# szbonaldo/FedMLP

Measured on AMD Instinct MI355X. Metric: images/sec/client (ICH 224x224 bs=128) at 1/2/4/8 GPUs; mAP vs ref, higher is better.
Workload: dtype f32; 1 GPU; FedMLP stage1 step, Resnet18, ICH-shaped synthetic 3x224x224, C=5, bs=128, one client per GPU, FedAvg all-reduce every 40 steps + once at end; parallelism=clients1, rccl_ranks=1, stream_mode=default: frozen teacher + weight gradients on the engine's side stream, arithmetic=fp32 operands+sums; products as 6 exact bf16 partials on the bf16 matrix pipe

## Files before the change

fedmlp_amd/_lib.py:

```python
import ctypes as C
import os

_HERE = os.path.dirname(os.path.abspath(__file__))
LIB_PATH = os.environ.get("FEDMLP_HIP_LIB") or os.path.join(_HERE, "libfedmlp_hip.so")

FM_MAX_CLASSES = 32
FM_COMM_ID_BYTES = 128


class FmConfig(C.Structure):
    _fields_ = [("model", C.c_int32), ("n_classes", C.c_int32), ("in_h", C.c_int32),
                ("in_w", C.c_int32), ("max_images", C.c_int32), ("reserved", C.c_int32 * 3),
                ("stream", C.c_void_p)]


class FmAdam(C.Structure):
    _fields_ = [("lr", C.c_float), ("beta1", C.c_float), ("beta2", C.c_float),
                ("eps", C.c_float), ("weight_decay", C.c_float)]


_P = C.c_void_p
_F = C.POINTER(C.c_float)
_I32 = C.c_int32
_I64 = C.c_int64
# ... 50 lines not shown
    "fm_profile_read": (C.c_int, [_P, _I32, C.POINTER(_I64), C.POINTER(C.c_double),
                                  C.POINTER(C.c_double)]),
    "fm_comm_preflight": (C.c_int, []),
    "fm_comm_unique_id": (C.c_int, [C.POINTER(C.c_uint8)]),
    "fm_comm_init": (C.c_int, [_P, C.POINTER(C.c_uint8), _I32, _I32]),
    "fm_comm_destroy": (C.c_int, [_P]),
    "fm_comm_size": (C.c_int, [_P]),
    "fm_fedavg_allreduce": (C.c_int, [_P, C.c_float]),
    "fm_fedavg_tao": (C.c_int, [_P, C.POINTER(C.c_double), C.c_double, _F, C.POINTER(C.c_double)]),
    "fm_fedavg_proto": (C.c_int, [_P, _P, C.c_double, _F, _P]),
    "fm_profile_ops": (C.c_int, [_P, _I32, C.c_char_p, _I32]),
    "fm_debug_num_convs": (C.c_int, [_P]),
    "fm_debug_conv_info": (C.c_int, [_P, _I32, C.POINTER(_I32)]),
    "fm_debug_conv": (C.c_int, [_P, _I32, _I32, _P, _P, _P, _I32, _I32, _P]),
    "fm_debug_block_dgrad": (C.c_int, [_P, _I32, _P, _P, _P, _I32]),
    "fm_debug_pw": (C.c_int, [_P, _I32, _I32, _P, _P, _P, _I32, _I32, _P, _P, _P, _P]),
    "fm_debug_proj_bwd": (C.c_int, [_P, _I32, _I32, _P, _P, _P, _P, _P, _I32, _I32, _P, _P]),
    "fm_debug_exp_bwd": (C.c_int, [_P, _I32, _P, _P, _P, _P, _P, _I32, _I32, _P, _P]),
    "fm_debug_get_grads": (C.c_int, [_P, _P]),
    "fm_debug_activation": (C.c_int, [_P, _I32, _I32, _I32, _P, C.POINTER(_I32)]),
    "fm_debug_stem_masks": (C.c_int, [_P, _I32, _I32, _P, _P]),
    "fm_debug_lose_part": (C.c_int, [_I32]),
    "fm_debug_ew": (C.c_int, [_P, _I32, C.POINTER(_P), C.POINTER(_I32), _F]),
    "fm_debug_eff": (C.c_int, [_P, _I32, C.POINTER(_P), C.POINTER(_I32), _F]),
    "fm_debug_eff_ws": (C.c_int, [_I32, C.POINTER(_I32), C.POINTER(C.c_int64)]),
}

_lib = None


# ... 39 lines not shown
```

fedmlp_amd/csrc/common.h:

```cpp
#pragma once
#include <hip/hip_runtime.h>
#include <stdint.h>

#include <stdlib.h>

typedef float f32x4 __attribute__((ext_vector_type(4)));

#ifndef FM_F32_FAST_SWISH
#define FM_F32_FAST_SWISH 1
#endif
#ifdef __HIPCC__
__device__ __forceinline__ float fm_swish_f32(float v)
{
#if FM_F32_FAST_SWISH
    return v * __builtin_amdgcn_rcpf(1.f + __expf(-v));
#else
    return v / (1.f + expf(-v));
#endif
}
#endif


#ifndef FM_MFMA_SPLIT_DEFAULT
#define FM_MFMA_SPLIT_DEFAULT 6
// ... 112 lines not shown
    int sp = 0;
    const unsigned short* Wsp = nullptr;
    const unsigned short* Xp = nullptr;
    long long xp_pix = 0;
    unsigned short* Yp = nullptr;
    long long yp_pix = 0;
    const unsigned short* resp = nullptr;
    int wrow = 0;
    int lose_part = 0;
    int* err = nullptr;
    int* err_host = nullptr;
    int njobs = 0;
    PconvJob job[PCONV_MAX_JOBS];
    const unsigned short* Xp2 = nullptr;
    unsigned wsp_bytes = 0;
};
void pconv_debug_lose_part(int on);

struct WgradParams {
    const float* dY;
    const float* X;
    float* slab;
    const int4* tab;
    const float* zeros;
    int M, Nw;
    int Ho, Wo, Hi, Wi, Ci, stride;
    int npix;
    int pix_per_split;
    int tilesM, tilesN;
    int bn;
// ... 23 lines not shown
    float* stats;
    int imgs, imgs_per_group, Hp, Wp, Ho, Wo, relu, sp;
    long long plane_bytes;
};
bool stem_rows_takes(int k, int stride, int cout, int hout, int wout, long long plane_bytes);
int stem_rows_stats_tiles(int imgs_per_group, int hout);
void launch_stem_rows(StemRowsParams p, hipStream_t s);
void k_stem_weight_planes(const float* w, unsigned short* dst, int Kw, hipStream_t s);
int launch_pwgrad(PwgradParams p, size_t slab_floats, hipStream_t s);
bool pwgrad_ring_takes(const PwgradParams& p);
int launch_pwgrad_ring(PwgradParams p, size_t slab_floats, hipStream_t s);
bool pwgrad_takes(int M, int Ci, int ksz, long long npix, long long xpix, int Wi, int pad);
void launch_igemm(IgemmParams p, int groups, hipStream_t s);
void launch_pconv(IgemmParams p, int groups, hipStream_t s);
bool pconv_takes(int M, int Ci, long long xp_pix, int Wi);
bool pconv_uses_ts(const IgemmParams& p);
int pconv_tile_m(int M);
int pconv_tile_n(int M);
size_t pconv_slab_floats();
bool launch_conv1x1_stream(const IgemmParams& p, int groups, hipStream_t s);
bool conv1x1_stream_takes(int Ci, int M, int Co);
int igemm_max_blocks();
bool launch_wgrad(const WgradParams& p, int splits, hipStream_t s);
int wgrad_tile_n(int M, int Nw);
int launch_wgrad_skinny(const WgradParams& p, size_t slab_floats, hipStream_t s);
int igemm_tile_n(int M, bool stem = false);
int igemm_tile_m(int M);

#include <stdio.h>
inline void set_max_dyn_lds(const void* fn, int bytes, const char* what)
// ... 5 lines not shown
```

fedmlp_amd/csrc/engine.hip:

```cpp
#include <math.h>
#include <stdio.h>
#include <string.h>

#include <algorithm>
#include <string>
#include <vector>

#include "../../include/fedmlp_hip.h"
#include "../../include/fedmlp_hip_debug.h"
#include "comm.h"
#include "common.h"
#include "kernels.h"
#include "pwconv.h"

static thread_local std::string g_err;
const char* fm_last_error(void) { return g_err.c_str(); }
const char* fm_version(void) { return "fedmlp_hip 0.2 (gfx950)"; }

#define HIPCHK(x)                                                                              \
    do {                                                                                       \
        hipError_t e_ = (x);                                                                   \
        if (e_ != hipSuccess) {                                                                \
            char b_[512];                                                                      \
            snprintf(b_, sizeof b_, "%s:%d %s -> %s", __FILE__, __LINE__, #x, hipGetErrorString(e_)); \
// ... 141 lines not shown
    size_t NP = 0, NS = 0;
    size_t off_fcw = 0, off_fcb = 0, off_gamma = 0, off_beta = 0, off_rm = 0, off_rv = 0;
    int64_t nf_sd = 0, ni_sd = 0;
    float *grad = nullptr, *adam_m = nullptr, *adam_v = nullptr;
    float* stage_sd = nullptr;
    fm_adam hp{3e-5f, 0.9f, 0.999f, 1e-8f, 5e-4f};
    int64_t adam_t = 0;
    float *x4 = nullptr, *dyh0 = nullptr;
    float* x3 = nullptr;
    bool stem_rows = false;
    unsigned short* x3p = nullptr;
    long long x3p_plane_elems = 0;
    uint8_t* idx0 = nullptr;
    float *GA = nullptr, *GB = nullptr, *GC = nullptr, *GD = nullptr, *GE = nullptr;
    float *ws_stats = nullptr, *ws_part = nullptr;
    int stats_conv = -1, stats_tiles_n = 0;
    size_t slab_floats = 0;
    float *ca = nullptr, *cb = nullptr, *cc = nullptr;
    float *feat = nullptr, *logits = nullptr, *tfeat = nullptr, *tlogits = nullptr, *dlogits = nullptr;
    float* psum = nullptr;
    int64_t *pcnt = nullptr, *tcnt = nullptr;
    float* zeros = nullptr;
    int *sel_counts = nullptr, *sel_top = nullptr, *sel_bot = nullptr, *cls_dev = nullptr;
    int sel_cap = 0;
    int* tag_buf = nullptr;
    size_t tag_buf_ints = 0;
    bool prof = false, prof_fail = false;
    hipError_t soft_err = hipSuccess;
    int* dev_err = nullptr;
    int* host_err = nullptr;
    int* host_err_dev = nullptr;
// ... 652 lines not shown
    const Conv& c0 = e->convs[0];
    if (e->model == 0) {
        const size_t pooled = B * (c0.hout / 2) * (c0.wout / 2) * 64;
        DALLOC(e->idx0, pooled);
        DALLOC(e->dyh0, B * c0.hout * c0.wout * 64);
        DALLOC(e->GA, pooled); DALLOC(e->GB, pooled); DALLOC(e->GC, pooled); DALLOC(e->GD, pooled); DALLOC(e->GE, pooled);
    } else {
        const EffSizes z = eff_sizes(e);
        AALLOC(e->GA, z.g_io); AALLOC(e->GB, z.g_io);
        AALLOC(e->T_small, z.t_small); AALLOC(e->T_big, z.t_big);
        DALLOC(e->se_dgp, B * z.max_ce); DALLOC(e->se_drp, B * z.max_cs); DALLOC(e->se_ds, B * z.max_ce);
        side = side && side_fits(e);
        DALLOC(e->hfeat, B * e->D);
    }
    DALLOC(e->ws_stats, max_stats);
    DALLOC(e->ws_part, (size_t)2 * (1024 + 32) * 2 * e->maxC);
    e->slab_floats = std::max<size_t>(max_slab * 8, (size_t)48 << 20);
    DALLOC(e->main.ws_slab, e->slab_floats);
    e->main.rec = e->main.ws_slab;
    DALLOC(e->ca, 2 * e->maxC); DALLOC(e->cb, 2 * e->maxC); DALLOC(e->cc, 2 * e->maxC);
    DALLOC(e->feat, B * e->D); DALLOC(e->tfeat, B * e->D);
    DALLOC(e->logits, B * e->C); DALLOC(e->tlogits, B * e->C); DALLOC(e->dlogits, B * e->C);
    DALLOC(e->psum, (size_t)2 * e->C * e->D); DALLOC(e->pcnt, 2 * e->C); DALLOC(e->tcnt, e->C);
    DALLOC(e->sel_counts, 2); DALLOC(e->cls_dev, FM_MAX_CLASSES);
    DALLOC(e->zeros, 64);
    if (e->planes) {
        const size_t pooled = B * (c0.hout / 2) * (c0.wout / 2) * 64;
        PALLOC(e->GBp, pooled); PALLOC(e->GCp, pooled); PALLOC(e->GDp, pooled);
        size_t mx = 0;
        for (auto& c : e->convs) {
            if (c.cin == 3) continue;
// ... 177 lines not shown
    p.imgs_per_group = imgs / groups;
    p.tilesM = (c.cout_p + igemm_tile_m(c.cout_p) - 1) / igemm_tile_m(c.cout_p);
    const int bn = igemm_tile_n(c.cout_p, c.cin == 3);
    p.tilesN = (p.imgs_per_group * c.hout * c.wout + bn - 1) / bn;
    p.relu = relu;
    ProfScope ps(e, L, c.cin == 3 ? 2 : (c.cout_p >= 128 ? 0 : 1), 2.0 * c.macs_per_img * imgs);
    launch_igemm(p, groups, L.st);
}

int stats_tiles(fm_engine* e, int ci)
{
    if (e->stats_conv != ci) soft(e, hipErrorInvalidValue);
    return e->stats_tiles_n;
}

void conv_dgrad(fm_engine* e, Lane& L, int ci, const float* dy, float* dx, int imgs, const float* res,
                bool acc_cls0, const unsigned short* dyp = nullptr)
{
    Conv& c = e->convs[ci];
    if (e->planes && c.ncls > 0 && c.cls[0].bm_off >= 0 &&
        pconv_takes(c.cin_p, c.cout_p, (long long)imgs * c.hout * c.wout, c.wout)) {
        const long long xp_pix = (long long)imgs * c.hout * c.wout;
        if (!dyp) dyp = scratch_planes(e, L, dy, xp_pix, c.cout_p);
        for (int k = 0; k < c.ncls; ++k) {
            DgradClass& d = c.cls[k];
            IgemmParams p{};
            p.Xp = dyp; p.xp_pix = xp_pix; p.Wsp = e->wbm_d + d.bm_off;
            p.Y = dx; p.slab = L.sk_slab; p.counters = L.sk_counters; p.err = e->dev_err; p.err_host = e->host_err_dev; p.sp = e->products;
            p.ntaps = d.taps.n;
            for (int t = 0; t < d.taps.n; ++t) { p.dh[t] = d.dh[t]; p.dw[t] = d.dw[t]; }
            p.res = res ? res : ((acc_cls0 && d.ph == 0 && d.pw == 0) ? dx : nullptr);
            p.M = c.cin_p;
            p.Hi = c.hout; p.Wi = c.wout; p.Ci = c.cout_p;
            p.Hg = (c.hin - d.ph + c.stride - 1) / c.stride;
            p.Wg = (c.win - d.pw + c.stride - 1) / c.stride;
            p.sg = 1;
            p.Ho = c.hin; p.Wo = c.win; p.Co = c.cin_p;
            p.os = c.stride; p.oh0 = d.ph; p.ow0 = d.pw;
            p.imgs_per_group = imgs;
            p.tilesM = c.cin_p / pconv_tile_m(c.cin_p);
            p.tilesN = (imgs * p.Hg * p.Wg + pconv_tile_n(c.cin_p) - 1) / pconv_tile_n(c.cin_p);
            p.relu = 0;
            ProfScope ps(e, L, (c.cin_p >= 128 ? 0 : 1) + (pconv_uses_ts(p) ? 0 : 6), 2.0 * c.macs_per_img * imgs * d.taps.n / (double)(c.k * c.k));
            launch_pconv(p, 1, L.st);
        }
        return;
    }
    if (e->planes && c.cin != 3) { soft(e, hipErrorInvalidValue); return; }
    if (e->precision && c.k == 1) {
        PwParams q{};
        q.zeros = e->zeros;
        q.W = e->student.wb + c.wbt_off;
        q.X = reinterpret_cast<const bf16*>(dy); q.Y = reinterpret_cast<bf16*>(dx);
        q.M = c.cin_p; q.K = c.cout_p;
        q.npix = imgs * c.hout * c.wout; q.groups = 1;
        q.res = reinterpret_cast<const bf16*>(res);
        q.HW = c.hout * c.wout;
        launch_pw_conv(q, L.st);
        return;
// ... 166 lines not shown
void bn_fwd_finalize(fm_engine* e, Lane& L, int ci, int groups, int imgs_per_group, BnMode mode)
{
    const Conv& c = e->convs[ci];
    const int bi = c.bn;
    Bn& b = e->bns[bi];
    if (mode == BnMode::Frozen) { bn_fwd_fixed(e, L, b, groups); return; }
    const bool run = mode == BnMode::Batch;
    k_bn_finalize(e->ws_stats, groups, stats_tiles(e, ci), b.C, imgs_per_group * c.hout * c.wout,
                  e->student.state + e->off_gamma + b.ch_off, e->student.state + e->off_beta + b.ch_off,
                  run ? e->student.state + e->off_rm + b.ch_off : nullptr, run ? e->student.state + e->off_rv + b.ch_off : nullptr, b.mean,
                  b.istd, b.scale, b.shift, e->bn_eps, e->bn_mom, L.st, e->dev_err);
    if (run) e->student.counters[bi] += groups;
}

void bn_bwd(fm_engine* e, Lane& L, int bi, const float* dz, const float* z, float* dy, float* dyh_out, int groups,
            int imgs_per_group, bool frozen, bool z_is_relu_of_bn = false, unsigned short* dyp = nullptr, const unsigned short* zh = nullptr)
{
    const Conv& c = e->convs[bi];
    Bn& b = e->bns[bi];
    const int pix = imgs_per_group * c.hout * c.wout;
    const char* fy = getenv("FM_BN_MASK_FROM_Y");
    const int from_y = fy ? atoi(fy) : 1;
    const float *msc = nullptr, *msh = nullptr;
    if (z_is_relu_of_bn && (z || zh) && (from_y || !z)) { msc = b.scale; msh = b.shift; z = nullptr; zh = nullptr; }
    k_bn_bwd_reduce(dz, z, c.y, b.mean, b.istd, e->ws_part, groups, pix, b.C, L.st, msc, msh, zh);
    k_bn_bwd_finalize(e->ws_part, groups, bn_bwd_blocks(pix), b.C, pix, e->student.state + e->off_gamma + b.ch_off, b.mean,
                      b.istd, e->ca, e->cb, e->cc, e->grad + e->off_gamma + b.ch_off,
                      e->grad + e->off_beta + b.ch_off, L.st, frozen);
    if (dyp) k_bn_bwd_apply_planes(dz, z, c.y, e->ca, e->cb, e->cc, dy, dyp, dyh_out, groups, pix, b.C, L.st, msc, msh, zh);
    else k_bn_bwd_apply(dz, z, c.y, e->ca, e->cb, e->cc, dy, dyh_out, groups, pix, b.C, L.st, msc, msh);
}

void to_nhwc4(fm_engine* e, Lane& L, const float* const* xs, int groups, int B)
{
    if (e->precision && e->model == 1) {
        const Conv& c = e->convs[e->c_stem];
        for (int g = 0; g < groups; ++g)
            k_stem_im2col(xs[g], reinterpret_cast<bf16*>(e->stem_col) + (size_t)g * B * c.hout * c.wout * c.Kw, B, e->H, e->W, c.hout,
                          c.wout, c.k, c.stride, c.pad, c.pad, L.st);
        return;
    }
// ... 215 lines not shown
    unsigned short* PB[2] = {e->GBp, sw ? e->GB2p : e->GBp};
    unsigned short* PC[2] = {e->GCp, sw ? e->GC2p : e->GCp};
    unsigned short* PD[2] = {e->GDp, sw ? e->GD2p : e->GDp};
    k_fc_bwd(e->dlogits, e->feat, S + e->off_fcw, nullptr, e->grad + e->off_fcw, e->grad + e->off_fcb, e->GA, DT_F32, imgs,
             512, e->C, cl.hout * cl.wout, L.st, bw.dfeat);
    float *ga = e->GA, *ge = e->GE;
    for (int b = (int)e->blocks.size() - 1; b >= 0; --b) {
        const Block& blk = e->blocks[b];
        const BlockActs& a = A.blk[b];
        const int par = b & 1;
        float *GB = GBp[par], *GC = GCp[par], *GD = GDp[par];
        unsigned short *gbp = pm ? PB[par] : nullptr, *gcp = pm ? PC[par] : nullptr, *gdp = pm ? PD[par] : nullptr;
        const float* in = b == 0 ? A.p0 : A.blk[b - 1].out;
        const bool last = b + 1 == (int)e->blocks.size();
        side_guard(e, 0, par);
        if (pm && !last) bn_bwd(e, L, blk.c2, ga, nullptr, nullptr, ga, groups, B, bw.frozen, false, gbp, a.outp);
        else bn_bwd(e, L, blk.c2, ga, a.out, pm ? nullptr : GB, ga, groups, B, bw.frozen, false, gbp);
        if (blk.ds >= 0) { side_guard(e, 1, par); bn_bwd(e, L, blk.ds, ga, nullptr, pm ? nullptr : GC, nullptr, groups, B, bw.frozen, false, gcp); }
        side_guard(e, 2, par);
        conv_dgrad(e, L, blk.c2, GB, GD, imgs, nullptr, false, gbp);
        conv_wgrad(e, side_begin(e, 0, par), blk.c2, a.z1, GB, imgs, nullptr, 0, pm ? a.z1p : nullptr, gbp);
        side_end(e, 0, par);
        if (pm) bn_bwd(e, L, blk.c1, GD, nullptr, nullptr, nullptr, groups, B, bw.frozen, true, gdp, a.z1p);
        else bn_bwd(e, L, blk.c1, GD, a.z1, GD, nullptr, groups, B, bw.frozen, true);
        if (blk.ds >= 0) {
            if (!block_dgrad(e, L, blk.c1, blk.ds, GD, GC, ge, imgs, gdp, gcp)) {
                conv_dgrad(e, L, blk.ds, GC, ge, imgs, nullptr, false, gcp);
                conv_dgrad(e, L, blk.c1, GD, ge, imgs, nullptr, true, gdp);
            }
        } else {
            conv_dgrad(e, L, blk.c1, GD, ge, imgs, ga, false, gdp);
        }
        const unsigned short* inp = pm ? (b == 0 ? A.p0p : A.blk[b - 1].outp) : nullptr;
        conv_wgrad(e, side_begin(e, 2, par), blk.c1, in, GD, imgs, nullptr, 0, inp, gdp);
        side_end(e, 2, par);
        if (blk.ds >= 0) {
            conv_wgrad(e, side_begin(e, 1, par), blk.ds, in, GC, imgs, nullptr, 0, inp, gcp);
            side_end(e, 1, par);
        }
        std::swap(ga, ge);
    }
    const Conv& c0 = e->convs[0];
    {
        Bn& b0 = e->bns[0];
// ... 1333 lines not shown
int fm_debug_block_dgrad(fm_engine* e, int32_t block, const float* dy1_dev, const float* dyd_dev, float* dx_dev, int32_t imgs)
{
    ARGCHK(e && dy1_dev && dyd_dev && dx_dev, "null tensor");
    ARGCHK(e->model == 0 && !e->precision, "fm_debug_block_dgrad: a precision-0 ResNet-18 engine");
    ARGCHK(block >= 0 && block < (int)e->blocks.size() && e->blocks[block].ds >= 0, "block has no downsample");
    ARGCHK(imgs >= 1 && imgs <= e->maxB, "imgs");
    ensure_packed(e);
    const Block& blk = e->blocks[block];
    if (!block_dgrad(e, e->main, blk.c1, blk.ds, dy1_dev, dyd_dev, dx_dev, imgs)) {
        conv_dgrad(e, e->main, blk.ds, dyd_dev, dx_dev, imgs, nullptr, false);
        conv_dgrad(e, e->main, blk.c1, dy1_dev, dx_dev, imgs, nullptr, true);
    }
    return FM_OK;
}

int fm_debug_conv_info(fm_engine* e, int32_t conv, int32_t* info16)
{
    ARGCHK(e && info16 && conv >= 0 && conv < (int)e->convs.size(), "conv index");
    const Conv& c = e->convs[conv];
    const int v[16] = {c.cin, c.cout, c.k, c.stride, c.pad, c.hin, c.win, c.hout, c.wout, c.cin_p, c.Kw, c.kw_p,
                       c.cout_p, 0, 0, 0};
    memcpy(info16, v, sizeof v);
    return FM_OK;
}

int fm_debug_conv(fm_engine* e, int32_t op, int32_t conv, const float* x_dev, const float* dy_dev, float* out_dev,
                  int32_t imgs, int32_t groups, float* stats_dev)
{
    ARGCHK(e && out_dev && conv >= 0 && conv < (int)e->convs.size(), "conv index");
    ARGCHK(!e->precision, "fm_debug_conv works on fp32 tensors: create the engine with precision 0");
// ... 264 lines not shown
```

fedmlp_amd/csrc/pconv.hip:

```cpp
#include <stdlib.h>

#include <algorithm>
#include <type_traits>

#include "common.h"
#include "kernels.h"
#include "split3.h"

#if __HIP_DEVICE_COMPILE__
template <int IMM> __device__ __forceinline__ sp_u32x4 pc_lds_read128(unsigned addr)
{
    sp_u32x4 v;
    asm volatile("ds_read_b128 %0, %1 offset:%2" : "=v"(v) : "v"(addr), "n"(IMM));
    return v;
}
__device__ __forceinline__ void pc_divmod(int x, int d, float rcp, int& q, int& r)
{
    q = (int)((float)x * rcp);
    r = x - q * d;
    if (r < 0) { --q; r += d; }
    else if (r >= d) { ++q; r -= d; }
}
template <int CTRL> __device__ __forceinline__ float pc_dpp(float v)
{
// ... 7 lines not shown
template <int SP> __device__ __forceinline__ f32x4 pc_mfma(const sp_u32x4 (&a)[3], const sp_u32x4 (&b)[3], f32x4 v)
{
    return mfma_split<SP>(a[0], a[1], a[2], b[0], b[1], b[2], v);
}
#endif

#ifdef PC_PHASES
__device__ unsigned long long pc_prof[256 * 8];
#define PC_T(i) do { const unsigned long long t_ = clock64(); pc_acc[i] += t_ - pc_t; pc_t = t_; } while (0)
#else
#define PC_T(i) do { } while (0)
#endif
#ifndef PC_WAVES_PER_EU
#define PC_WAVES_PER_EU 2
#endif
template <int FR, int FC, int NS, int SP, bool TS = false>
__global__ __launch_bounds__(512, PC_WAVES_PER_EU) void pconv_kernel(const IgemmParams p)
{
#if __HIP_DEVICE_COMPILE__
#ifdef PC_PHASES
    unsigned long long pc_acc[8] = {0, 0, 0, 0, 0, 0, 0, 0};
    unsigned long long pc_t = clock64();
#endif
    constexpr int WN = 4;
    constexpr int BM = 32 * FR, BN = 64 * FC;
    constexpr int GA = BM / 16, GB = TS ? (BN + 2 + 15) / 16 : BN / 16;
    constexpr int BROWS = 16 * GB;
    constexpr int SA = 3 * BM * 64, SB = 3 * BROWS * 64;
    constexpr int NSB = TS ? 2 : NS;
    static_assert(!TS || FC == 4, "tap-row sharing: 256-pixel tiles");
    constexpr int JA = (3 * GA + 7) / 8;
    constexpr int RGB = (GB + 7) / 8;
    static_assert(NS == 2 && FC == 4 && (FR == 2 || FR == 4), "two LDS stages, 256-pixel tiles, 64 or 128 rows");
    typedef __attribute__((address_space(3))) void lds_void;
    extern __shared__ __attribute__((aligned(16))) unsigned char smem[];
    const int tid = threadIdx.x;
    const int lane = tid & 63, wave = __builtin_amdgcn_readfirstlane(tid >> 6);
    const int wm = wave / WN, wn = wave % WN;
    const int li = lane & 15, lg = lane >> 4;
    const unsigned lds0 = (unsigned)(size_t)smem;
    const unsigned As = lds0, Bs = lds0 + NS * SA;

    const int Wi = p.Wi;
    struct JobV {
        int nsteps, ntaps, k2, icc2;
// ... 431 lines not shown
                            for (int c = 0; c < FC; ++c)
                                part[q][c] = *reinterpret_cast<const f32x4*>(src + (((r + q) * FC + c) * 512 + tid) * 4);
#pragma unroll
                        for (int q = 0; q < 2; ++q)
#pragma unroll
                            for (int c = 0; c < FC; ++c) acc[r + q][c] += part[q][c];
                    }
                }
            }
        }

        PC_T(5);
        if (do_epilogue) {
        const int mbase = m0 + wm * (16 * FR) + 4 * lg;
        const JobV J = jobv(cur.jb);
        if (p.stats) {
            float* red = fsmem;
#pragma unroll
            for (int r = 0; r < FR; ++r) {
                f32x4 s1 = {0.f, 0.f, 0.f, 0.f}, s2 = {0.f, 0.f, 0.f, 0.f};
#pragma unroll
                for (int c = 0; c < FC; ++c) {
                    s1 += acc[r][c];
                    s2 += acc[r][c] * acc[r][c];
                }
#pragma unroll
                for (int q = 0; q < 4; ++q) {
                    float u = s1[q], v = s2[q];
                    u += pc_dpp<0xB1>(u); v += pc_dpp<0xB1>(v);
                    u += pc_dpp<0x4E>(u); v += pc_dpp<0x4E>(v);
                    u += pc_dpp<0x12C>(u); v += pc_dpp<0x12C>(v);
// ... 17 lines not shown
                st[m0 + ch] = u;
                st[p.M + m0 + ch] = v;
            }
        }
        size_t opix[FC];
        bool ok[FC];
#pragma unroll
        for (int c = 0; c < FC; ++c) {
            const int n = n0 + wn * (16 * FC) + 16 * c + li;
            ok[c] = n < J.npix;
            int img, rem, hg, wg;
            pc_divmod(ok[c] ? n : J.npix - 1, J.HWg, J.rcpHW, img, rem);
            pc_divmod(rem, J.Wg, J.rcpW, hg, wg);
            opix[c] = (size_t)((grp * p.imgs_per_group + img) * p.Ho + hg * p.os + J.oh0) * p.Wo + (wg * p.os + J.ow0);
        }
#pragma unroll
        for (int r = 0; r < FR; r += 2) {
            __builtin_amdgcn_sched_barrier(0);
            const int m = mbase + 16 * r;
            const size_t cb = (size_t)(m0 + wm * (16 * FR) + 16 * r) >> 5;
            f32x4 sc0 = {1.f, 1.f, 1.f, 1.f}, sc1 = sc0, sh0 = {0.f, 0.f, 0.f, 0.f}, sh1 = sh0;
            if (p.scale) {
                sc0 = *reinterpret_cast<const f32x4*>(p.scale + m); sc1 = *reinterpret_cast<const f32x4*>(p.scale + m + 16);
                sh0 = *reinterpret_cast<const f32x4*>(p.shift + m); sh1 = *reinterpret_cast<const f32x4*>(p.shift + m + 16);
            }
#pragma unroll
            for (int c = 0; c < FC; ++c) {
                __builtin_amdgcn_sched_barrier(0);
                const size_t o = opix[c] * p.Co;
                f32x4 v0 = acc[r][c], v1 = acc[r + 1][c];
// ... 23 lines not shown
                }
                if (!ok[c]) continue;
                if (p.Y) {
                    *reinterpret_cast<f32x4*>(p.Y + o + m) = v0;
                    *reinterpret_cast<f32x4*>(p.Y + o + m + 16) = v1;
                }
                if (p.Yp) {
                    sp_u32x4 H, M, L;
                    split3(v0, v1, H, M, L);
                    unsigned char* dst = reinterpret_cast<unsigned char*>(p.Yp) + ((cb * 3) * (size_t)p.yp_pix + opix[c]) * 64 + lg * 16;
                    *reinterpret_cast<sp_u32x4*>(dst) = H;
                    *reinterpret_cast<sp_u32x4*>(dst + (size_t)p.yp_pix * 64) = M;
                    *reinterpret_cast<sp_u32x4*>(dst + (size_t)p.yp_pix * 128) = L;
                }
            }
        }
        }
        PC_T(6);
        if (!more) break;
        PC_SYNC_LDS();
        cur = nx;
    }
    if (pend_tile >= 0) {
        asm volatile("s_waitcnt vmcnt(0)" ::: "memory");
        __syncthreads();
        if (tid == 0) {
            __builtin_amdgcn_fence(__ATOMIC_RELEASE, "agent");
            asm volatile("s_waitcnt vmcnt(0)" ::: "memory");
            if (!p.lose_part) __hip_atomic_fetch_add(p.counters + pend_tile, 1, __ATOMIC_RELAXED, __HIP_MEMORY_SCOPE_AGENT);
        }
// ... 77 lines not shown
    return ((long long)(Ci >> 5) * 3 * xp_pix + Wi + 1) * 64 < 0x7ff00000LL && xp_pix < (1LL << 22);
}

bool pconv_uses_ts(const IgemmParams& p)
{
    bool ts = p.njobs == 0 && p.ntaps == 9 && p.sg == 1 && p.Hg == p.Hi && p.Wg == p.Wi;
    for (int j = 0; ts && j < 3; ++j) {
        ts = p.dh[3 * j] == p.dh[3 * j + 1] && p.dh[3 * j] == p.dh[3 * j + 2];
        int seen = 0;
        for (int k = 0; k < 3; ++k) seen |= 1 << (p.dw[3 * j + k] + 1);
        ts = ts && seen == 7;
    }
    return ts;
}

void launch_pconv(IgemmParams p, int groups, hipStream_t s)
{
    static bool attr_done = false;
    constexpr int LDS_L = 2 * 3 * (128 + 256) * 64 + 4 * 128 * 2 * 4;
    constexpr int LDS_S = 2 * 3 * (64 + 256) * 64 + 4 * 128 * 2 * 4;
    constexpr int LDS_LT = 2 * 3 * 128 * 64 + 2 * 3 * 272 * 64 + 4 * 128 * 2 * 4;
    constexpr int LDS_ST = 2 * 3 * 64 * 64 + 2 * 3 * 272 * 64 + 4 * 128 * 2 * 4;
    if (!attr_done) {
        set_max_dyn_lds(reinterpret_cast<const void*>(&pconv_kernel<4, 4, 2, 6, true>), LDS_LT, "pconv_kernel<4, 4, 2, 6, true>");
        set_max_dyn_lds(reinterpret_cast<const void*>(&pconv_kernel<4, 4, 2, 9, true>), LDS_LT, "pconv_kernel<4, 4, 2, 9, true>");
        set_max_dyn_lds(reinterpret_cast<const void*>(&pconv_kernel<2, 4, 2, 6, true>), LDS_ST, "pconv_kernel<2, 4, 2, 6, true>");
        set_max_dyn_lds(reinterpret_cast<const void*>(&pconv_kernel<2, 4, 2, 9, true>), LDS_ST, "pconv_kernel<2, 4, 2, 9, true>");
        set_max_dyn_lds(reinterpret_cast<const void*>(&pconv_kernel<4, 4, 2, 6>), LDS_L, "pconv_kernel<4, 4, 2, 6>");
        set_max_dyn_lds(reinterpret_cast<const void*>(&pconv_kernel<4, 4, 2, 9>), LDS_L, "pconv_kernel<4, 4, 2, 9>");
        set_max_dyn_lds(reinterpret_cast<const void*>(&pconv_kernel<2, 4, 2, 6>), LDS_S, "pconv_kernel<2, 4, 2, 6>");
        set_max_dyn_lds(reinterpret_cast<const void*>(&pconv_kernel<2, 4, 2, 9>), LDS_S, "pconv_kernel<2, 4, 2, 9>");
        attr_done = true;
    }
    const bool ts = pconv_uses_ts(p);
    p.tapcode = pconv_tapcode(p.dh, p.dw, p.ntaps);
    if (p.njobs == 0) {
        p.njobs = 1;
        PconvJob& j = p.job[0];
        j.ntaps = p.ntaps; j.tapcode = p.tapcode;
        j.cib = j.icc2 = p.Ci >> 5; j.wofs = j.wofs2 = 0;
        j.Hg = p.Hg; j.Wg = p.Wg; j.oh0 = p.oh0; j.ow0 = p.ow0;
    }
// ... 18 lines not shown
    p.tn_fast = p.tilesM > 1 && (long long)p.M * p.nsteps * 192 > (3LL << 20);
    static const int forced = getenv("FM_IGEMM_BLOCKS") ? atoi(getenv("FM_IGEMM_BLOCKS")) : 0;
    int nblk = p.total_steps >= 4LL * pconv_max_blocks() ? pconv_max_blocks() : (int)std::min<long long>(pconv_max_blocks(), T);
    if (forced > 0) nblk = (int)std::min<long long>(std::min(forced, pconv_max_blocks()), p.total_steps);
    p.steps_per_block = (int)((p.total_steps + nblk - 1) / nblk);
    if (forced <= 0 && p.steps_per_block > p.nsteps / 2 && (long long)p.nsteps * 128 * 192 > (2LL << 20)) {
        for (int P = 1; P <= 12; ++P) {
            if (p.nsteps % P) continue;
            const int q = p.nsteps / P;
            const int sq = (p.steps_per_block + q - 1) / q * q;
            if ((long long)sq * 100 <= (long long)p.steps_per_block * 102) { p.steps_per_block = sq; break; }
        }
    }
    dim3 grid(nblk);
    p.lose_part = g_lose_part ? 1 : 0;
    if (ts) {
        if (p.M >= 128) {
            if (p.sp == 9) hipLaunchKernelGGL((pconv_kernel<4, 4, 2, 9, true>), grid, dim3(512), LDS_LT, s, p);
            else hipLaunchKernelGGL((pconv_kernel<4, 4, 2, 6, true>), grid, dim3(512), LDS_LT, s, p);
        } else {
            if (p.sp == 9) hipLaunchKernelGGL((pconv_kernel<2, 4, 2, 9, true>), grid, dim3(512), LDS_ST, s, p);
            else hipLaunchKernelGGL((pconv_kernel<2, 4, 2, 6, true>), grid, dim3(512), LDS_ST, s, p);
        }
        return;
    }
    if (p.M >= 128) {
        if (p.sp == 9) hipLaunchKernelGGL((pconv_kernel<4, 4, 2, 9>), grid, dim3(512), LDS_L, s, p);
        else hipLaunchKernelGGL((pconv_kernel<4, 4, 2, 6>), grid, dim3(512), LDS_L, s, p);
    } else {
        if (p.sp == 9) hipLaunchKernelGGL((pconv_kernel<2, 4, 2, 9>), grid, dim3(512), LDS_S, s, p);
// ... 34 lines not shown
```

fedmlp_amd/engine.py:

```python
import ctypes as C

import numpy as np
import torch

from . import _lib, spec

MODEL_IDS = {"Resnet18": 0, "Efficient_b0": 1}
PRECISION_IDS = {"fp32": 0, "bf16": 1}
PRODUCT_FORMS = {None: 0, 6: 3, 0: 1, 9: 2}


def _ptr(t):
    if t is None:
        return None
    assert t.is_cuda and t.is_contiguous() and t.dtype in (torch.float32, torch.int32, torch.bfloat16), \
        (t.device, t.dtype, t.is_contiguous())
    return C.c_void_p(t.data_ptr())


class Engine:

    def __init__(self, model, n_classes, in_h, in_w, max_images, device=None, precision="fp32", streams=0, products=None):
        if not torch.cuda.is_available():
            raise RuntimeError("fedmlp_amd.Engine needs a GPU (no CPU fallback)")
# ... 433 lines not shown
        _lib.check(self.lib.fm_debug_activation(self.h, kind, block, imgs, out.ctypes.data_as(C.c_void_p), dims))
        return np.ascontiguousarray(out.transpose(0, 3, 1, 2))

    def debug_num_convs(self):
        return self.lib.fm_debug_num_convs(self.h)

    def debug_conv(self, op, conv, x, dy, out, imgs, groups=1, stats=None):
        self._enqueue()
        _lib.check(self.lib.fm_debug_conv(self.h, op, conv, _ptr(x), _ptr(dy), _ptr(out), imgs, groups,
                                          _ptr(stats)))

    def debug_block_dgrad(self, block, dy1, dyd, dx, imgs):
        self._enqueue()
        _lib.check(self.lib.fm_debug_block_dgrad(self.h, block, _ptr(dy1), _ptr(dyd), _ptr(dx), imgs))

    EW_OPS = ("split_planes", "planes_to_f32", "bn_finalize", "bn_finalize_frozen", "bn_eval_affine", "bn_apply",
              "bn_apply_planes", "stem_pool", "stem_pool_planes", "stem_pool_bwd", "stem_pool_bn_reduce", "stem_pool_bn_apply",
              "bn_bwd_reduce", "bn_bwd_finalize", "bn_bwd_apply", "bn_bwd_apply_planes")

    def debug_ew(self, op, ptrs, dims, scalars=()):
        assert len(ptrs) <= 12 and len(dims) <= 5 and len(scalars) <= 2, (len(ptrs), len(dims), len(scalars))
        for t in ptrs:
            assert t is None or (t.is_cuda and t.is_contiguous()), op
        p = (C.c_void_p * 12)(*[None if t is None else t.data_ptr() for t in ptrs])
        d = (C.c_int32 * 5)(*[int(v) for v in dims])
        _lib.check(self.lib.fm_debug_ew(self.h, self.EW_OPS.index(op), p, d, _lib.fvec(list(scalars) + [0.0] * (2 - len(scalars)))))

    EFF_OPS = ("dw_fwd", "dw_dgrad", "dw_wgrad", "se_fwd", "se_scale", "se_bwd_bn1", "se_wgrad")

    def debug_eff_ws(self, op, dims):
# ... 61 lines not shown
```

include/fedmlp_hip_debug.h:

```cpp
#ifndef FEDMLP_HIP_DEBUG_H
#define FEDMLP_HIP_DEBUG_H

#include "fedmlp_hip.h"

#ifdef __cplusplus
extern "C" {
#endif

int fm_debug_conv_info(fm_engine* e, int32_t conv, int32_t* info16);
int fm_debug_num_convs(fm_engine* e);
int fm_debug_conv(fm_engine* e, int32_t op, int32_t conv, const float* x_dev, const float* dy_dev,
                  float* out_dev, int32_t imgs, int32_t groups, float* stats_dev);

int fm_debug_block_dgrad(fm_engine* e, int32_t block, const float* dy1_dev, const float* dyd_dev, float* dx_dev, int32_t imgs);

int fm_debug_pw(fm_engine* e, int32_t op, int32_t conv, const void* x_dev, const void* dy_dev, void* out_dev,
                int32_t imgs, int32_t groups, const float* psc_dev, const float* psh_dev, const float* gate_dev,
                float* stats_dev);

int fm_debug_proj_bwd(fm_engine* e, int32_t conv, int32_t phase, const void* dyp_dev, const void* yd_dev, const float* bn_dev,
                      const float* gate_dev, const float* ds_dev, int32_t imgs, int32_t groups, void* out_dev,
                      float* pool5_dev);

int fm_debug_exp_bwd(fm_engine* e, int32_t conv, const void* da_dev, const void* ye_dev, const void* x_dev, const void* res_dev,
                     const float* bn_dev, int32_t imgs, int32_t groups, void* dx_dev, float* dw_dev);

int fm_debug_activation(fm_engine* e, int32_t kind, int32_t block, int32_t imgs, float* host_nhwc,
                        int32_t* dims4);

// ... 28 lines not shown
```

Measured before the change: 6174 images/sec.

## Fuse BatchNorm backward channel sums into tap-sharing dgrad epilogue

The planes-mode data-gradient convolution now computes, in its epilogue, the per-channel BatchNorm backward partial sums (sum of masked dz and sum of dz times normalized y) for the following BN layer and writes them to the partial workspace. The separate bn_bwd_reduce pass is then skipped, and finalize reads the tile-level partials. This removes one full read of the gradient and activation tensors per block, at the cost of extra loads and cross-lane reductions in the conv epilogue, more register pressure, and eight new kernel instantiations. Residual-add blocks take their ReLU mask from the stored planes.

```diff
diff --git a/fedmlp_amd/_lib.py b/fedmlp_amd/_lib.py
--- a/fedmlp_amd/_lib.py
+++ b/fedmlp_amd/_lib.py
@@ -88,6 +88,9 @@
     "fm_debug_conv_info": (C.c_int, [_P, _I32, C.POINTER(_I32)]),
     "fm_debug_conv": (C.c_int, [_P, _I32, _I32, _P, _P, _P, _I32, _I32, _P]),
     "fm_debug_block_dgrad": (C.c_int, [_P, _I32, _P, _P, _P, _I32]),
+    "fm_debug_dgrad_sums": (C.c_int, [_P, _I32, _I32, _I32, _P, _P, _P, _P, _P, _P, _P, _P, _P, _P, _I64, _I32, _I32,
+                                      C.POINTER(_I32)]),
+    "fm_debug_bn_sums": (C.c_int, [_P, _I32]),
     "fm_debug_pw": (C.c_int, [_P, _I32, _I32, _P, _P, _P, _I32, _I32, _P, _P, _P, _P]),
     "fm_debug_proj_bwd": (C.c_int, [_P, _I32, _I32, _P, _P, _P, _P, _P, _I32, _I32, _P, _P]),
     "fm_debug_exp_bwd": (C.c_int, [_P, _I32, _P, _P, _P, _P, _P, _I32, _I32, _P, _P]),
diff --git a/fedmlp_amd/csrc/common.h b/fedmlp_amd/csrc/common.h
--- a/fedmlp_amd/csrc/common.h
+++ b/fedmlp_amd/csrc/common.h
@@ -150,6 +150,14 @@
     PconvJob job[PCONV_MAX_JOBS];
     const unsigned short* Xp2 = nullptr;
     unsigned wsp_bytes = 0;
+    int bs_mode = 0;
+    const float* bs_y = nullptr;
+    const float* bs_mean = nullptr;
+    const float* bs_istd = nullptr;
+    const float* bs_msc = nullptr;
+    const float* bs_msh = nullptr;
+    const unsigned short* bs_zh = nullptr;
+    float* bs_part = nullptr;
 };
 void pconv_debug_lose_part(int on);
 
@@ -203,6 +211,7 @@
 void launch_igemm(IgemmParams p, int groups, hipStream_t s);
 void launch_pconv(IgemmParams p, int groups, hipStream_t s);
 bool pconv_takes(int M, int Ci, long long xp_pix, int Wi);
+bool pconv_takes_sums(const IgemmParams& p);
 bool pconv_uses_ts(const IgemmParams& p);
 int pconv_tile_m(int M);
 int pconv_tile_n(int M);
diff --git a/fedmlp_amd/csrc/engine.hip b/fedmlp_amd/csrc/engine.hip
--- a/fedmlp_amd/csrc/engine.hip
+++ b/fedmlp_amd/csrc/engine.hip
@@ -179,7 +179,10 @@
     uint8_t* idx0 = nullptr;
     float *GA = nullptr, *GB = nullptr, *GC = nullptr, *GD = nullptr, *GE = nullptr;
     float *ws_stats = nullptr, *ws_part = nullptr;
+    size_t ws_part_floats = 0;
     int stats_conv = -1, stats_tiles_n = 0;
+    int part_bn = -1, part_tiles_n = 0;
+    bool bn_sums = true;
     size_t slab_floats = 0;
     float *ca = nullptr, *cb = nullptr, *cc = nullptr;
     float *feat = nullptr, *logits = nullptr, *tfeat = nullptr, *tlogits = nullptr, *dlogits = nullptr;
@@ -862,7 +865,8 @@
         DALLOC(e->hfeat, B * e->D);
     }
     DALLOC(e->ws_stats, max_stats);
-    DALLOC(e->ws_part, (size_t)2 * (1024 + 32) * 2 * e->maxC);
+    e->ws_part_floats = (size_t)2 * (1024 + 32) * 2 * e->maxC;
+    DALLOC(e->ws_part, e->ws_part_floats);
     e->slab_floats = std::max<size_t>(max_slab * 8, (size_t)48 << 20);
     DALLOC(e->main.ws_slab, e->slab_floats);
     e->main.rec = e->main.ws_slab;
@@ -1070,10 +1074,26 @@
     return e->stats_tiles_n;
 }
 
+struct DgradSums {
+    int bn, groups;
+    const float *y, *mean, *istd, *msc, *msh;
+    const unsigned short* zh;
+    float* part;
+    size_t part_floats;
+};
+DgradSums dgrad_sums_for(fm_engine* e, int bi, int groups, const unsigned short* zh)
+{
+    const Bn& b = e->bns[bi];
+    return DgradSums{bi, groups, e->convs[bi].y, b.mean, b.istd, zh ? nullptr : b.scale, zh ? nullptr : b.shift, zh, e->ws_part,
+                     e->ws_part_floats};
+}
+int part_tiles(fm_engine* e, int bi) { return e->part_bn == bi ? e->part_tiles_n : 0; }
+
 void conv_dgrad(fm_engine* e, Lane& L, int ci, const float* dy, float* dx, int imgs, const float* res,
-                bool acc_cls0, const unsigned short* dyp = nullptr)
+                bool acc_cls0, const unsigned short* dyp = nullptr, const DgradSums* sums = nullptr)
 {
     Conv& c = e->convs[ci];
+    if (sums) e->part_bn = -1;
     if (e->planes && c.ncls > 0 && c.cls[0].bm_off >= 0 &&
         pconv_takes(c.cin_p, c.cout_p, (long long)imgs * c.hout * c.wout, c.wout)) {
         const long long xp_pix = (long long)imgs * c.hout * c.wout;
@@ -1097,8 +1117,23 @@
             p.tilesM = c.cin_p / pconv_tile_m(c.cin_p);
             p.tilesN = (imgs * p.Hg * p.Wg + pconv_tile_n(c.cin_p) - 1) / pconv_tile_n(c.cin_p);
             p.relu = 0;
+            int groups = 1;
+            if (sums && c.ncls == 1 && imgs % sums->groups == 0) {
+                IgemmParams q = p;
+                q.imgs_per_group = imgs / sums->groups;
+                q.tilesN = (q.imgs_per_group * p.Hg * p.Wg + pconv_tile_n(c.cin_p) - 1) / pconv_tile_n(c.cin_p);
+                q.bs_mode = sums->zh ? 2 : 1;
+                q.bs_y = sums->y; q.bs_mean = sums->mean; q.bs_istd = sums->istd; q.bs_part = sums->part;
+                q.bs_msc = sums->msc; q.bs_msh = sums->msh;
+                if (sums->zh) { q.bs_zh = sums->zh; q.yp_pix = (long long)imgs * c.hin * c.win; }
+                const size_t need = (size_t)sums->groups * (q.tilesN + (q.tilesN > 64 ? 32 : 0)) * 2 * c.cin_p;
+                if (need <= sums->part_floats && pconv_takes_sums(q)) {
+                    p = q; groups = sums->groups;
+                    e->part_bn = sums->bn; e->part_tiles_n = q.tilesN;
+                }
+            }
             ProfScope ps(e, L, (c.cin_p >= 128 ? 0 : 1) + (pconv_uses_ts(p) ? 0 : 6), 2.0 * c.macs_per_img * imgs * d.taps.n / (double)(c.k * c.k));
-            launch_pconv(p, 1, L.st);
+            launch_pconv(p, groups, L.st);
         }
         return;
     }
@@ -1295,7 +1330,8 @@
 }
 
 void bn_bwd(fm_engine* e, Lane& L, int bi, const float* dz, const float* z, float* dy, float* dyh_out, int groups,
-            int imgs_per_group, bool frozen, bool z_is_relu_of_bn = false, unsigned short* dyp = nullptr, const unsigned short* zh = nullptr)
+            int imgs_per_group, bool frozen, bool z_is_relu_of_bn = false, unsigned short* dyp = nullptr, const unsigned short* zh = nullptr,
+            int sums_ready = 0)
 {
     const Conv& c = e->convs[bi];
     Bn& b = e->bns[bi];
@@ -1304,8 +1340,9 @@
     const int from_y = fy ? atoi(fy) : 1;
     const float *msc = nullptr, *msh = nullptr;
     if (z_is_relu_of_bn && (z || zh) && (from_y || !z)) { msc = b.scale; msh = b.shift; z = nullptr; zh = nullptr; }
-    k_bn_bwd_reduce(dz, z, c.y, b.mean, b.istd, e->ws_part, groups, pix, b.C, L.st, msc, msh, zh);
-    k_bn_bwd_finalize(e->ws_part, groups, bn_bwd_blocks(pix), b.C, pix, e->student.state + e->off_gamma + b.ch_off, b.mean,
+    if (!sums_ready) k_bn_bwd_reduce(dz, z, c.y, b.mean, b.istd, e->ws_part, groups, pix, b.C, L.st, msc, msh, zh);
+    e->part_bn = -1;
+    k_bn_bwd_finalize(e->ws_part, groups, sums_ready ? sums_ready : bn_bwd_blocks(pix), b.C, pix, e->student.state + e->off_gamma + b.ch_off, b.mean,
                       b.istd, e->ca, e->cb, e->cc, e->grad + e->off_gamma + b.ch_off,
                       e->grad + e->off_beta + b.ch_off, L.st, frozen);
     if (dyp) k_bn_bwd_apply_planes(dz, z, c.y, e->ca, e->cb, e->cc, dy, dyp, dyh_out, groups, pix, b.C, L.st, msc, msh, zh);
@@ -1551,20 +1588,26 @@
         const float* in = b == 0 ? A.p0 : A.blk[b - 1].out;
         const bool last = b + 1 == (int)e->blocks.size();
         side_guard(e, 0, par);
-        if (pm && !last) bn_bwd(e, L, blk.c2, ga, nullptr, nullptr, ga, groups, B, bw.frozen, false, gbp, a.outp);
+        if (pm && !last) bn_bwd(e, L, blk.c2, ga, nullptr, nullptr, ga, groups, B, bw.frozen, false, gbp, a.outp, part_tiles(e, blk.c2));
         else bn_bwd(e, L, blk.c2, ga, a.out, pm ? nullptr : GB, ga, groups, B, bw.frozen, false, gbp);
         if (blk.ds >= 0) { side_guard(e, 1, par); bn_bwd(e, L, blk.ds, ga, nullptr, pm ? nullptr : GC, nullptr, groups, B, bw.frozen, false, gcp); }
         side_guard(e, 2, par);
-        conv_dgrad(e, L, blk.c2, GB, GD, imgs, nullptr, false, gbp);
+        const bool sums = pm && e->bn_sums && !bw.frozen;
+        const DgradSums s1 = dgrad_sums_for(e, blk.c1, groups, nullptr);
+        conv_dgrad(e, L, blk.c2, GB, GD, imgs, nullptr, false, gbp, sums ? &s1 : nullptr);
         conv_wgrad(e, side_begin(e, 0, par), blk.c2, a.z1, GB, imgs, nullptr, 0, pm ? a.z1p : nullptr, gbp);
         side_end(e, 0, par);
-        if (pm) bn_bwd(e, L, blk.c1, GD, nullptr, nullptr, nullptr, groups, B, bw.frozen, true, gdp, a.z1p);
+        if (pm) bn_bwd(e, L, blk.c1, GD, nullptr, nullptr, nullptr, groups, B, bw.frozen, true, gdp, a.z1p, part_tiles(e, blk.c1));
         else bn_bwd(e, L, blk.c1, GD, a.z1, GD, nullptr, groups, B, bw.frozen, true);
         if (blk.ds >= 0) {
             if (!block_dgrad(e, L, blk.c1, blk.ds, GD, GC, ge, imgs, gdp, gcp)) {
                 conv_dgrad(e, L, blk.ds, GC, ge, imgs, nullptr, false, gcp);
                 conv_dgrad(e, L, blk.c1, GD, ge, imgs, nullptr, true, gdp);
             }
+        } else if (b > 0) {
+            const int c2b = e->blocks[b - 1].c2;
+            const DgradSums s2 = dgrad_sums_for(e, c2b, groups, A.blk[b - 1].outp);
+            conv_dgrad(e, L, blk.c1, GD, ge, imgs, ga, false, gdp, sums ? &s2 : nullptr);
         } else {
             conv_dgrad(e, L, blk.c1, GD, ge, imgs, ga, false, gdp);
         }
@@ -2928,6 +2971,41 @@
     return FM_OK;
 }
 
+int fm_debug_dgrad_sums(fm_engine* e, int32_t conv, int32_t H, int32_t W, const float* dy_dev, const float* res_dev, const float* y_dev,
+                        const float* mean_dev, const float* istd_dev, const float* mask_scale_dev, const float* mask_shift_dev,
+                        const uint16_t* zh_dev, float* dx_dev, float* part_dev, int64_t part_floats, int32_t imgs, int32_t groups,
+                        int32_t* tiles_out)
+{
+    ARGCHK(e && dy_dev && y_dev && mean_dev && istd_dev && dx_dev && part_dev && tiles_out, "null operand");
+    ARGCHK(e->model == 0 && e->planes, "fm_debug_dgrad_sums: a planes-mode ResNet-18 engine");
+    ARGCHK(conv >= 0 && conv < (int)e->convs.size(), "conv index");
+    Conv& c = e->convs[conv];
+    ARGCHK(c.k == 3 && c.stride == 1 && c.ncls == 1, "a 3x3 / stride-1 convolution");
+    ARGCHK(imgs >= 1 && groups >= 1 && imgs % groups == 0 && H >= 1 && W >= 1 && H <= c.hin && W <= c.win &&
+               (long long)imgs * H * W <= (long long)e->maxB * c.hin * c.win, "imgs / groups / H / W");
+    ARGCHK(zh_dev ? (res_dev && !mask_scale_dev && !mask_shift_dev) : (!res_dev && mask_scale_dev && mask_shift_dev),
+           "mask from y: scale + shift and no residual; mask from planes: zh + the residual");
+    ensure_packed(e);
+    const Conv saved = c;
+    c.hin = c.hout = H; c.win = c.wout = W;
+    const DgradSums ds{-1, groups, y_dev, mean_dev, istd_dev, mask_scale_dev, mask_shift_dev, zh_dev, part_dev, (size_t)part_floats};
+    e->part_tiles_n = 0;
+    conv_dgrad(e, e->main, conv, dy_dev, dx_dev, imgs, res_dev, false, nullptr, &ds);
+    c = saved;
+    *tiles_out = e->part_tiles_n;
+    e->part_bn = -1;
+    HIPCHK(hipStreamSynchronize(e->main.st));
+    ARGCHK(*tiles_out > 0, "the launch could not carry the sums (shape, or part too small)");
+    return FM_OK;
+}
+
+int fm_debug_bn_sums(fm_engine* e, int32_t on)
+{
+    ARGCHK(e, "null engine");
+    e->bn_sums = on != 0;
+    return FM_OK;
+}
+
 int fm_debug_conv_info(fm_engine* e, int32_t conv, int32_t* info16)
 {
     ARGCHK(e && info16 && conv >= 0 && conv < (int)e->convs.size(), "conv index");
diff --git a/fedmlp_amd/csrc/pconv.hip b/fedmlp_amd/csrc/pconv.hip
--- a/fedmlp_amd/csrc/pconv.hip
+++ b/fedmlp_amd/csrc/pconv.hip
@@ -45,7 +45,7 @@
 #ifndef PC_WAVES_PER_EU
 #define PC_WAVES_PER_EU 2
 #endif
-template <int FR, int FC, int NS, int SP, bool TS = false>
+template <int FR, int FC, int NS, int SP, bool TS = false, int BS = 0>
 __global__ __launch_bounds__(512, PC_WAVES_PER_EU) void pconv_kernel(const IgemmParams p)
 {
 #if __HIP_DEVICE_COMPILE__
@@ -60,6 +60,7 @@
     constexpr int SA = 3 * BM * 64, SB = 3 * BROWS * 64;
     constexpr int NSB = TS ? 2 : NS;
     static_assert(!TS || FC == 4, "tap-row sharing: 256-pixel tiles");
+    static_assert(BS == 0 || TS, "BatchNorm sums: the tap-sharing data gradients");
     constexpr int JA = (3 * GA + 7) / 8;
     constexpr int RGB = (GB + 7) / 8;
     static_assert(NS == 2 && FC == 4 && (FR == 2 || FR == 4), "two LDS stages, 256-pixel tiles, 64 or 128 rows");
@@ -521,7 +522,7 @@
         if (do_epilogue) {
         const int mbase = m0 + wm * (16 * FR) + 4 * lg;
         const JobV J = jobv(cur.jb);
-        if (p.stats) {
+        if (BS == 0 && p.stats) {
             float* red = fsmem;
 #pragma unroll
             for (int r = 0; r < FR; ++r) {
@@ -569,6 +570,88 @@
             pc_divmod(rem, J.Wg, J.rcpW, hg, wg);
             opix[c] = (size_t)((grp * p.imgs_per_group + img) * p.Ho + hg * p.os + J.oh0) * p.Wo + (wg * p.os + J.ow0);
         }
+        if constexpr (BS != 0) {
+            float* red = fsmem;
+#pragma unroll
+            for (int r = 0; r < FR; r += 2) {
+                __builtin_amdgcn_sched_barrier(0);
+                const int m = mbase + 16 * r;
+                const size_t cb = (size_t)(m0 + wm * (16 * FR) + 16 * r) >> 5;
+                const size_t gm = (size_t)grp * p.M + m;
+                const f32x4 mu0 = *reinterpret_cast<const f32x4*>(p.bs_mean + gm), mu1 = *reinterpret_cast<const f32x4*>(p.bs_mean + gm + 16);
+                const f32x4 is0 = *reinterpret_cast<const f32x4*>(p.bs_istd + gm), is1 = *reinterpret_cast<const f32x4*>(p.bs_istd + gm + 16);
+                f32x4 sc0 = {0.f, 0.f, 0.f, 0.f}, sc1 = sc0, sh0 = sc0, sh1 = sc0;
+                if constexpr (BS == 1) {
+                    sc0 = *reinterpret_cast<const f32x4*>(p.bs_msc + gm); sc1 = *reinterpret_cast<const f32x4*>(p.bs_msc + gm + 16);
+                    sh0 = *reinterpret_cast<const f32x4*>(p.bs_msh + gm); sh1 = *reinterpret_cast<const f32x4*>(p.bs_msh + gm + 16);
+                }
+                f32x4 s1a = {0.f, 0.f, 0.f, 0.f}, s1b = s1a, s2a = s1a, s2b = s1a;
+#pragma unroll
+                for (int c = 0; c < FC; ++c) {
+                    __builtin_amdgcn_sched_barrier(0);
+                    const size_t o = opix[c] * p.Co;
+                    const f32x4 y0 = *reinterpret_cast<const f32x4*>(p.bs_y + o + m), y1 = *reinterpret_cast<const f32x4*>(p.bs_y + o + m + 16);
+                    f32x4 v0 = acc[r][c], v1 = acc[r + 1][c];
+                    bool k0[4], k1[4];
+                    if constexpr (BS == 1) {
+#pragma unroll
+                        for (int q = 0; q < 4; ++q) {
+                            k0[q] = __builtin_fmaf(y0[q], sc0[q], sh0[q]) > 0.f;
+                            k1[q] = __builtin_fmaf(y1[q], sc1[q], sh1[q]) > 0.f;
+                        }
+                    } else {
+                        const f32x4 a = *reinterpret_cast<const f32x4*>(p.res + o + m), b = *reinterpret_cast<const f32x4*>(p.res + o + m + 16);
+                        const sp_u32x4 H = *reinterpret_cast<const sp_u32x4*>(
+                            reinterpret_cast<const unsigned char*>(p.bs_zh) + ((cb * 3) * (size_t)p.yp_pix + opix[c]) * 64 + lg * 16);
+                        v0 += a; v1 += b;
+#pragma unroll
+                        for (int i = 0; i < 2; ++i) {
+                            k0[2 * i] = (short)(H[i] & 0xffffu) > 0; k0[2 * i + 1] = (short)(H[i] >> 16) > 0;
+                            k1[2 * i] = (short)(H[2 + i] & 0xffffu) > 0; k1[2 * i + 1] = (short)(H[2 + i] >> 16) > 0;
+                        }
+                    }
+                    f32x4 d0, d1;
+#pragma unroll
+                    for (int q = 0; q < 4; ++q) {
+                        d0[q] = (k0[q] && ok[c]) ? v0[q] : 0.f;
+                        d1[q] = (k1[q] && ok[c]) ? v1[q] : 0.f;
+                    }
+                    s1a += d0; s1b += d1;
+                    s2a += d0 * ((y0 - mu0) * is0); s2b += d1 * ((y1 - mu1) * is1);
+                    if (ok[c]) {
+                        *reinterpret_cast<f32x4*>(p.Y + o + m) = v0;
+                        *reinterpret_cast<f32x4*>(p.Y + o + m + 16) = v1;
+                    }
+                }
+#pragma unroll
+                for (int h = 0; h < 2; ++h)
+#pragma unroll
+                    for (int q = 0; q < 4; ++q) {
+                        float u = h ? s1b[q] : s1a[q], v = h ? s2b[q] : s2a[q];
+                        u += pc_dpp<0xB1>(u); v += pc_dpp<0xB1>(v);
+                        u += pc_dpp<0x4E>(u); v += pc_dpp<0x4E>(v);
+                        u += pc_dpp<0x12C>(u); v += pc_dpp<0x12C>(v);
+                        u += pc_dpp<0x128>(u); v += pc_dpp<0x128>(v);
+                        if (li == 0) {
+                            const int ml = wm * (16 * FR) + 16 * (r + h) + 4 * lg + q;
+                            red[(wn * BM + ml) * 2 + 0] = u;
+                            red[(wn * BM + ml) * 2 + 1] = v;
+                        }
+                    }
+            }
+            PC_SYNC_LDS();
+            for (int ch = tid; ch < BM; ch += 512) {
+                float u = 0.f, v = 0.f;
+#pragma unroll
+                for (int ww = 0; ww < WN; ++ww) {
+                    u += red[(ww * BM + ch) * 2 + 0];
+                    v += red[(ww * BM + ch) * 2 + 1];
+                }
+                float* st = p.bs_part + (size_t)(grp * J.tilesN + tn) * 2 * p.M;
+                st[m0 + ch] = u;
+                st[p.M + m0 + ch] = v;
+            }
+        } else {
 #pragma unroll
         for (int r = 0; r < FR; r += 2) {
             __builtin_amdgcn_sched_barrier(0);
@@ -622,6 +705,7 @@
                     *reinterpret_cast<sp_u32x4*>(dst + (size_t)p.yp_pix * 128) = L;
                 }
             }
+        }
         }
         }
         PC_T(6);
@@ -729,6 +813,15 @@
     return ts;
 }
 
+bool pconv_takes_sums(const IgemmParams& p)
+{
+    if (!pconv_uses_ts(p) || !p.Y || p.Yp || p.resp || p.scale || p.stats || p.relu || p.os != 1 || p.oh0 || p.ow0 || p.Co != p.M ||
+        p.Ho != p.Hg || p.Wo != p.Wg || !p.bs_y || !p.bs_mean || !p.bs_istd || !p.bs_part)
+        return false;
+    if (p.bs_mode == 1) return p.bs_msc && p.bs_msh && !p.res;
+    return p.bs_mode == 2 && p.bs_zh && p.res && p.yp_pix > 0;
+}
+
 void launch_pconv(IgemmParams p, int groups, hipStream_t s)
 {
     static bool attr_done = false;
@@ -741,6 +834,14 @@
         set_max_dyn_lds(reinterpret_cast<const void*>(&pconv_kernel<4, 4, 2, 9, true>), LDS_LT, "pconv_kernel<4, 4, 2, 9, true>");
         set_max_dyn_lds(reinterpret_cast<const void*>(&pconv_kernel<2, 4, 2, 6, true>), LDS_ST, "pconv_kernel<2, 4, 2, 6, true>");
         set_max_dyn_lds(reinterpret_cast<const void*>(&pconv_kernel<2, 4, 2, 9, true>), LDS_ST, "pconv_kernel<2, 4, 2, 9, true>");
+        set_max_dyn_lds(reinterpret_cast<const void*>(&pconv_kernel<4, 4, 2, 6, true, 1>), LDS_LT, "pconv_kernel<4, 4, 2, 6, true, 1>");
+        set_max_dyn_lds(reinterpret_cast<const void*>(&pconv_kernel<4, 4, 2, 9, true, 1>), LDS_LT, "pconv_kernel<4, 4, 2, 9, true, 1>");
+        set_max_dyn_lds(reinterpret_cast<const void*>(&pconv_kernel<2, 4, 2, 6, true, 1>), LDS_ST, "pconv_kernel<2, 4, 2, 6, true, 1>");
+        set_max_dyn_lds(reinterpret_cast<const void*>(&pconv_kernel<2, 4, 2, 9, true, 1>), LDS_ST, "pconv_kernel<2, 4, 2, 9, true, 1>");
+        set_max_dyn_lds(reinterpret_cast<const void*>(&pconv_kernel<4, 4, 2, 6, true, 2>), LDS_LT, "pconv_kernel<4, 4, 2, 6, true, 2>");
+        set_max_dyn_lds(reinterpret_cast<const void*>(&pconv_kernel<4, 4, 2, 9, true, 2>), LDS_LT, "pconv_kernel<4, 4, 2, 9, true, 2>");
+        set_max_dyn_lds(reinterpret_cast<const void*>(&pconv_kernel<2, 4, 2, 6, true, 2>), LDS_ST, "pconv_kernel<2, 4, 2, 6, true, 2>");
+        set_max_dyn_lds(reinterpret_cast<const void*>(&pconv_kernel<2, 4, 2, 9, true, 2>), LDS_ST, "pconv_kernel<2, 4, 2, 9, true, 2>");
         set_max_dyn_lds(reinterpret_cast<const void*>(&pconv_kernel<4, 4, 2, 6>), LDS_L, "pconv_kernel<4, 4, 2, 6>");
         set_max_dyn_lds(reinterpret_cast<const void*>(&pconv_kernel<4, 4, 2, 9>), LDS_L, "pconv_kernel<4, 4, 2, 9>");
         set_max_dyn_lds(reinterpret_cast<const void*>(&pconv_kernel<2, 4, 2, 6>), LDS_S, "pconv_kernel<2, 4, 2, 6>");
@@ -789,6 +890,22 @@
     }
     dim3 grid(nblk);
     p.lose_part = g_lose_part ? 1 : 0;
+    if (p.bs_mode) {
+#define PC_LAUNCH_BS(MODE)                                                                                                   \
+        do {                                                                                                                 \
+            if (p.M >= 128) {                                                                                                \
+                if (p.sp == 9) hipLaunchKernelGGL((pconv_kernel<4, 4, 2, 9, true, MODE>), grid, dim3(512), LDS_LT, s, p);  \
+                else hipLaunchKernelGGL((pconv_kernel<4, 4, 2, 6, true, MODE>), grid, dim3(512), LDS_LT, s, p);            \
+            } else {                                                                                                         \
+                if (p.sp == 9) hipLaunchKernelGGL((pconv_kernel<2, 4, 2, 9, true, MODE>), grid, dim3(512), LDS_ST, s, p);  \
+                else hipLaunchKernelGGL((pconv_kernel<2, 4, 2, 6, true, MODE>), grid, dim3(512), LDS_ST, s, p);            \
+            }                                                                                                                \
+        } while (0)
+        if (p.bs_mode == 1) PC_LAUNCH_BS(1);
+        else PC_LAUNCH_BS(2);
+#undef PC_LAUNCH_BS
+        return;
+    }
     if (ts) {
         if (p.M >= 128) {
             if (p.sp == 9) hipLaunchKernelGGL((pconv_kernel<4, 4, 2, 9, true>), grid, dim3(512), LDS_LT, s, p);
diff --git a/fedmlp_amd/engine.py b/fedmlp_amd/engine.py
--- a/fedmlp_amd/engine.py
+++ b/fedmlp_amd/engine.py
@@ -471,6 +471,20 @@
         self._enqueue()
         _lib.check(self.lib.fm_debug_block_dgrad(self.h, block, _ptr(dy1), _ptr(dyd), _ptr(dx), imgs))
 
+    def debug_dgrad_sums(self, conv, H, W, dy, y, mean, istd, dx, part, imgs, groups, res=None, mask_scale=None, mask_shift=None,
+                         zh=None):
+        self._enqueue()
+        for t in (dy, y, mean, istd, dx, part, res, mask_scale, mask_shift, zh):
+            assert t is None or (t.is_cuda and t.is_contiguous())
+        q = lambda t: None if t is None else C.c_void_p(t.data_ptr())
+        tiles = C.c_int32(0)
+        _lib.check(self.lib.fm_debug_dgrad_sums(self.h, conv, H, W, q(dy), q(res), q(y), q(mean), q(istd), q(mask_scale),
+                                                q(mask_shift), q(zh), q(dx), q(part), part.numel(), imgs, groups, C.byref(tiles)))
+        return tiles.value
+
+    def debug_bn_sums(self, on):
+        _lib.check(self.lib.fm_debug_bn_sums(self.h, int(bool(on))))
+
     EW_OPS = ("split_planes", "planes_to_f32", "bn_finalize", "bn_finalize_frozen", "bn_eval_affine", "bn_apply",
               "bn_apply_planes", "stem_pool", "stem_pool_planes", "stem_pool_bwd", "stem_pool_bn_reduce", "stem_pool_bn_apply",
               "bn_bwd_reduce", "bn_bwd_finalize", "bn_bwd_apply", "bn_bwd_apply_planes")
diff --git a/include/fedmlp_hip_debug.h b/include/fedmlp_hip_debug.h
--- a/include/fedmlp_hip_debug.h
+++ b/include/fedmlp_hip_debug.h
@@ -13,6 +13,12 @@
                   float* out_dev, int32_t imgs, int32_t groups, float* stats_dev);
 
 int fm_debug_block_dgrad(fm_engine* e, int32_t block, const float* dy1_dev, const float* dyd_dev, float* dx_dev, int32_t imgs);
+
+int fm_debug_dgrad_sums(fm_engine* e, int32_t conv, int32_t H, int32_t W, const float* dy_dev, const float* res_dev, const float* y_dev,
+                        const float* mean_dev, const float* istd_dev, const float* mask_scale_dev, const float* mask_shift_dev,
+                        const uint16_t* zh_dev, float* dx_dev, float* part_dev, int64_t part_floats, int32_t imgs, int32_t groups,
+                        int32_t* tiles_out);
+int fm_debug_bn_sums(fm_engine* e, int32_t on);
 
 int fm_debug_pw(fm_engine* e, int32_t op, int32_t conv, const void* x_dev, const void* dy_dev, void* out_dev,
                 int32_t imgs, int32_t groups, const float* psc_dev, const float* psh_dev, const float* gate_dev,
```

Result: no change. 6209 images/sec (median of 6 runs) (+0.6%).
